# vlad17/runlmc

Hardware: AMD Instinct MI355X
Metric: kronecker_toeplitz_mvms_per_sec (higher is better)
Workload: dtype f64

## Files before the change

### runlmc_amd/csrc/rl_filter.h

```cpp
#pragma once
#include "rl_device.h"

#define RL_SF_G 512
#define RL_SF_NH (RL_SF_G / 256)
#define RL_SF_S 32
#define RL_SF_LPR (RL_SF_G / RL_SF_S)
#define RL_SF_PAD (RL_SF_G + RL_SF_LPR)
#define RL_SF_NSEG 32
#define RL_SF_MAXTOPS 16
#define RL_SF_TOL 2e-14

__device__ __forceinline__ int sf_pad(int i) { return i + (i >> 5); }

struct SfTop {
    double rho;
    double c[4];
    double rG;
    double rL;
};

struct SfParams {
    int NF, nfac;
    const SfTop* tops;
    const double* pw;
    const double* kappa;
    const double* facA;
    const double* facAW;
    const int* facJ;
    const double* pwp;
};

template <int NS>
__device__ __forceinline__ double sf_step(double (&F)[NS], double rho, double x) {
    const double tt = rho * F[0];
// ... 659 lines not shown
        const bool shifted = gi > m - 2;
#pragma unroll
        for (int k = 0; k < XR / 2; ++k)
            if (k < D) {
                const double p0 = shifted ? xr[2 * k + 1] : xr[2 * k];
                xs[(size_t)k * PAD + pi] = gi < m ? p0 : 0.0;
                xs[(size_t)k * PAD + pi + 1] = gi + 1 < m ? xr[2 * k + 1] : 0.0;
            }
    }
#pragma unroll
    for (int k = 0; k < 4; ++k)
        if (tid + 256 * k < ncin) cinl[tid + 256 * k] = cr[k];
    RL_SF_STAMP(101);
    if (nfac > 0) {
#pragma unroll
        for (int half = 0; half < NH; ++half) {
            const int pi = sf_pad(2 * tid) + half;
            double xb[D];
#pragma unroll
            for (int b = 0; b < D; ++b) xb[b] = xs[(size_t)b * PAD + pi];
            for (int f = 0; f < nfac; ++f) {
                const double* ar = facA + f * D;
                double u = 0.0;
#pragma unroll
                for (int b = 0; b < D; ++b) u = fma(ar[b], xb[b], u);
                us[(size_t)f * PAD + pi] = u;
            }
        }
    }
    sf_lds_barrier();
    RL_SF_STAMP(102);
}

template <int NS, int D>
static __global__ void __launch_bounds__(256) RL_SF_APPLY_ATTR
k_sf_apply(const double* __restrict__ X, double* __restrict__ Y, int nvec, int m, int NF,
           int nfac, const double* __restrict__ blob, const double* __restrict__ Cin,
           int* __restrict__ next_tile) {
    constexpr int G = RL_SF_G, PAD = RL_SF_PAD, NH = RL_SF_NH, XR = NH * D, S = RL_SF_S;
    constexpr int B2 = NS < 4 ? 2 : 1;
    RL_SMEM(smem);
    const int nchan = D * NF + nfac, nblob = sf_blob_doubles(NF, nfac, D);
    double* xs = reinterpret_cast<double*>(smem);
    double* us = xs + (size_t)D * PAD;
    double* tab = us + (size_t)nfac * PAD;
    const double* kap = tab;
    const double* facA = kap + NF * D;
    const double* facAW = facA + nfac * D;
    const double* facJ = facAW + nfac * D;
    const SfBlk* bl = reinterpret_cast<const SfBlk*>(facJ + nfac);
    double* cinl = tab + nblob;
    int* nxt = reinterpret_cast<int*>(cinl + (size_t)nchan * 2 * NS);
    double* scr = cinl + (size_t)nchan * 2 * NS + 1;
    const int tid = threadIdx.x, nthr = blockDim.x, lane = tid & 63, wave = tid >> 6;
    const int nwaves = nthr >> 6;
    RL_CENSUS_ENTER(120);
#if defined(RL_TIMING) && !defined(RL_EMU)
    const long long sf_t0 = wall_clock64();
#endif
    for (int e = tid; e < nblob; e += nthr) tab[e] = blob[e];
    sf_lds_barrier();
    const int nch = (m + G - 1) / G, ntiles = nch * nvec, ncin = nchan * 2 * NS;
    int tile = blockIdx.x, sf_iter = -1;
    if (tid == 0) nxt[0] = (int)gridDim.x + atomicAdd(next_tile, 1);
    if (tile < ntiles) {
        double xr[XR], cr[4];
        sf_request<XR>(xr, cr, X, Cin, tile, nch, nvec, D, m, ncin, tid);
        RL_SF_STAMP(100);
        sf_stage<D, XR>(xr, cr, xs, us, cinl, facA, nfac, ncin, (tile % nch) * G, m, tid, sf_iter);
    }
    int slot = 0;
    while (tile < ntiles) {
    const int chunk = tile % nch, v = tile / nch, g0 = chunk * G;
    ++sf_iter;
    RL_SF_STAMP(99);
    for (int t0 = 0; t0 < D * 16; t0 += nthr) {
#if !defined(RL_EMU)
        if (t0 + wave * 64 >= D * 16) break;
#endif
        const int t = t0 + tid, araw = t >> 4, s = t & 15;
#if defined(RL_EMU)
        const bool live = araw < D;
#else
        if (araw >= D) continue;
        constexpr bool live = true;
#endif
        const int a = live ? araw : D - 1;
        double* cell = xs + (size_t)a * PAD + s * (S + 1);
        double xv[S];
#pragma unroll
        for (int i = 0; i < S; ++i) xv[i] = cell[i];
        for (int j = 0; j < NF;) {
            const int b = (NS == 2 && NF - j >= 5) ? 5 : (NF - j >= B2 ? B2 : 1);
            const double* kw = kap + j * D + a;
            const double* cin0 = cinl + (size_t)(a * NF + j) * 2 * NS;
            if (j == 0) {
                if (NS == 2 && b == 5) sf_task<2, 5, true>(cell, xv, live, s, bl, j, kw, D, cin0, scr);
                else if (b == 2) sf_task<NS, B2, true>(cell, xv, live, s, bl, j, kw, D, cin0, scr);
                else sf_task<NS, 1, true>(cell, xv, live, s, bl, j, kw, D, cin0, scr);
            } else {
                if (NS == 2 && b == 5) sf_task<2, 5, false>(cell, xv, live, s, bl, j, kw, D, cin0, scr);
                else if (b == 2) sf_task<NS, B2, false>(cell, xv, live, s, bl, j, kw, D, cin0, scr);
                else sf_task<NS, 1, false>(cell, xv, live, s, bl, j, kw, D, cin0, scr);
            }
            j += b;
        }
    }
    RL_SF_STAMP(103);
    const int next = nxt[slot];
    double xr[XR], cr[4];
#if defined(RL_EMU)
    for (int k = 0; k < XR; ++k) xr[k] = 0.0;
    for (int k = 0; k < 4; ++k) cr[k] = 0.0;
#endif
    if (next < ntiles) sf_request<XR>(xr, cr, X, Cin, next, nch, nvec, D, m, ncin, tid);
    RL_SF_STAMP(104);
    const int xw = (D * 16 + 63) / 64, uw0 = xw < nwaves ? xw : 0, nuw = nwaves - uw0;
    for (int t0 = 0; t0 < nfac * 16; t0 += nuw * 64) {
        const int t = t0 + (wave - uw0) * 64 + lane, fraw = t >> 4, s = t & 15;
#if defined(RL_EMU)
        const bool live = wave >= uw0 && fraw < nfac;
#else
        if (wave < uw0 || fraw >= nfac) continue;
        constexpr bool live = true;
#endif
        const int f = live ? fraw : 0;
        double* cell = us + (size_t)f * PAD + s * (S + 1);
        double xv[S];
#pragma unroll
        for (int i = 0; i < S; ++i) xv[i] = cell[i];
        sf_task<NS, 1, true>(cell, xv, live, s, bl, (int)facJ[f], nullptr, 0,
                             cinl + (size_t)(D * NF + f) * 2 * NS, scr);
    }
    RL_SF_STAMP(110);
    sf_lds_barrier();
    RL_SF_STAMP(111);
    slot ^= 1;
    int drawn = 0;
    if (tid == 0 && next < ntiles) drawn = (int)gridDim.x + atomicAdd(next_tile, 1);
    {
        const double* gAW = facAW;
        const int i0 = 2 * tid, pi = sf_pad(i0);
        double* ybase = Y + (size_t)v * D * m + g0 + i0;
        double acc[NH][D];
#pragma unroll
        for (int half = 0; half < NH; ++half) {
#pragma unroll
            for (int a = 0; a < D; ++a) acc[half][a] = xs[(size_t)a * PAD + pi + half];
            for (int f = 0; f < nfac; ++f) {
                const double* ar = gAW + f * D;
                const double uw = us[(size_t)f * PAD + pi + half];
#pragma unroll
                for (int a = 0; a < D; ++a) acc[half][a] = fma(ar[a], uw, acc[half][a]);
            }
        }
        if (g0 + i0 + 1 < m) {
#pragma unroll
            for (int a = 0; a < D; ++a)
                *reinterpret_cast<SfPair*>(ybase + (size_t)a * m) = SfPair{acc[0][a], acc[1][a]};
        } else if (g0 + i0 < m) {
#pragma unroll
            for (int a = 0; a < D; ++a) ybase[(size_t)a * m] = acc[0][a];
        }
    }
    RL_SF_STAMP(112);
    if (tid == 0) nxt[slot] = drawn;
    tile = next;
    if (tile < ntiles) {
        RL_SF_STAMP(100);
        sf_stage<D, XR>(xr, cr, xs, us, cinl, facA, nfac, ncin, (tile % nch) * G, m, tid, sf_iter);
    }
    }
    RL_CENSUS_LEAVE(120);
#if defined(RL_TIMING) && !defined(RL_EMU)
    if (threadIdx.x == 0) {
        const unsigned long long d = (unsigned long long)(wall_clock64() - sf_t0);
        atomicMax((unsigned long long*)&rl_timing_buf[210], d);
        atomicAdd((unsigned long long*)&rl_timing_buf[211], d);
        atomicAdd((unsigned long long*)&rl_timing_buf[212], 1ull);
        atomicMax((unsigned long long*)&rl_timing_buf[213], (1ull << 40) - d);
    }
#endif
}
```

### runlmc_amd/csrc/rl_gridop.hip

```cpp
#include "rl_host.h"

static thread_local std::string g_err;

int fail(int code, const std::string& msg) {
    g_err = msg;
    return code;
}

extern "C" const char* rl_last_error(void) { return g_err.c_str(); }
extern "C" const char* rl_backend(void) { return RL_BACKEND_NAME; }
extern "C" int rl_abi_version(void) { return RL_ABI_VERSION; }
extern "C" int rl_device_count(int* count) {
    if (!count) return fail(RL_EINVAL, "count is NULL");
    RL_HIP(hipGetDeviceCount(count));
    return RL_OK;
}

void trace_once(const char* what) {
    static const bool on = getenv("RUNLMC_TRACE") != nullptr;
    if (!on) return;
    static std::vector<std::string> seen;
    for (const std::string& s : seen)
        if (s == what) return;
    seen.push_back(what);
// ... 29 lines not shown
        if (getenv(n) == nullptr) return false;
        if (!debug) ignored(n);
        return debug;
    };
    auto num = [&](const char* n, long long dflt) {
        const char* e = getenv(n);
        if (e == nullptr) return dflt;
        if (!debug) ignored(n);
        return debug ? atoll(e) : dflt;
    };
    k.pow2_only = user_flag("RUNLMC_POW2_ONLY");
    k.chunk_mb = (int)num("RUNLMC_CHUNK_MB", 0);
    k.two_streams = (int)num("RUNLMC_TWO_STREAMS", -1);
    k.affine = (int)num("RUNLMC_AFFINE", -1);
    k.affine_kb = (int)num("RUNLMC_AFFINE_KB", 0);
    k.affine_max_kb = (int)num("RUNLMC_AFFINE_MAX_KB", 2048);
    k.no_v1p = flag("RUNLMC_NO_V1P");
    k.v1p_min = (int)num("RUNLMC_V1P_MIN", 0);
    k.no_lowrank = flag("RUNLMC_NO_LOWRANK");
    k.no_filter = flag("RUNLMC_NO_FILTER");
    k.no_lr_bound = flag("RUNLMC_NO_LR_BOUND");
    k.sf_carries1 = flag("RUNLMC_SF_CARRIES1");
    k.sf_scan2 = flag("RUNLMC_SF_SCAN2");
    k.poly_round = flag("RUNLMC_POLY_ROUND");
    k.no_poly_round = flag("RUNLMC_NO_POLY_ROUND");
    k.lr_min = num("RUNLMC_LR_MIN", -1);
    k.staged_wt = flag("RUNLMC_STAGED_WT");
    k.no_staged_wt = flag("RUNLMC_NO_STAGED_WT");
    k.no_w_poly = flag("RUNLMC_NO_W_POLY");
    k.no_rp = flag("RUNLMC_NO_RP");
    k.rp_stagger = (int)num("RUNLMC_RP_STAGGER", 7);
    k.no_lr_small = flag("RUNLMC_NO_LR_SMALL");
    k.lr_expand_plain = (int)num("RUNLMC_LR_EXPAND_PLAIN", 0);
    k.no_precond_approx = flag("RUNLMC_NO_PRECOND_APPROX");
    k.no_precond_hi = flag("RUNLMC_NO_PRECOND_HI");
    k.precond_hi_passes = flag("RUNLMC_PRECOND_HI_PASSES");
    k.no_precond_hi_mixed = flag("RUNLMC_NO_PRECOND_HI_MIXED");
    k.precond_hi_min = num("RUNLMC_PRECOND_HI_MIN", 100000);
    k.precond_hi_rank = (int)num("RUNLMC_PRECOND_HI_RANK", 192);
    k.precond_hi_use = (int)num("RUNLMC_PRECOND_HI_USE", 0);
    k.rp_fly = (int)num("RUNLMC_RP_FLY", 1);
    k.no_rp_small = flag("RUNLMC_NO_RP_SMALL");
    k.no_rp_fuse = flag("RUNLMC_NO_RP_FUSE");
    k.rp_pfuse = !flag("RUNLMC_NO_RP_PFUSE");
    k.w_pfuse = !flag("RUNLMC_NO_W_PFUSE");
    k.rp_runlen = (int)num("RUNLMC_RP_RUNLEN", 0);
    k.w_poly_rmax = std::min(36, (int)num("RUNLMC_W_POLY_RMAX", 32));
    k.no_sort = flag("RUNLMC_NO_SORT");
    k.ws_cache_mb = user_num("RUNLMC_WS_CACHE_MB", -1);
    k.solver_maxblk = (int)num("RUNLMC_SOLVER_MAXBLK", 0);
    k.no_fuse_w = flag("RUNLMC_NO_FUSE_W");
    k.no_fuse_wt = flag("RUNLMC_NO_FUSE_WT");
    k.no_graph = flag("RUNLMC_NO_GRAPH");
#if defined(RL_EMU)
    k.minres_v1 = flag("RUNLMC_MINRES_V1");
#endif
    return k;
}

static int ilog2(int x) {
    int l = 0;
    while ((1 << l) < x) ++l;
    return l;
}

static FftPlan make_plan(int n) {
// ... 168 lines not shown
}

static void set_lds_attrs() {
#if !defined(RL_EMU)
    static unsigned long long seen = 0;
    if (!first_on_device(&seen)) return;
    (void)hipFuncSetAttribute((const void*)k_cols_fwd,
                              hipFuncAttributeMaxDynamicSharedMemorySize, 160 * 1024);
    (void)hipFuncSetAttribute((const void*)k_cols_inv,
                              hipFuncAttributeMaxDynamicSharedMemorySize, 160 * 1024);
    (void)hipFuncSetAttribute((const void*)k_rows_spec,
                              hipFuncAttributeMaxDynamicSharedMemorySize, 160 * 1024);
    set_lds_attr_cols2<8, 8>(); set_lds_attr_cols2<8, 16>(); set_lds_attr_cols2<16, 16>();
    set_lds_attr_cols2<3, 8>(); set_lds_attr_cols2<3, 16>();
    set_lds_attr_cols2<5, 8>(); set_lds_attr_cols2<5, 16>();
    set_lds_attr_rows<1>();  set_lds_attr_rows<2>();  set_lds_attr_rows<3>();
    set_lds_attr_rows<4>();  set_lds_attr_rows<5>();  set_lds_attr_rows<6>();
    set_lds_attr_rows<7>();  set_lds_attr_rows<8>();  set_lds_attr_rows<9>();
    set_lds_attr_rows<10>(); set_lds_attr_rows<11>(); set_lds_attr_rows<12>();
    set_lds_attr_rows<13>(); set_lds_attr_rows<14>(); set_lds_attr_rows<15>();
    set_lds_attr_rows<16>();
    set_lds_attr_rows3<1>();  set_lds_attr_rows3<2>();  set_lds_attr_rows3<3>();
    set_lds_attr_rows3<4>();  set_lds_attr_rows3<5>();  set_lds_attr_rows3<6>();
    set_lds_attr_rows3<7>();  set_lds_attr_rows3<8>();  set_lds_attr_rows3<9>();
    set_lds_attr_rows3<10>(); set_lds_attr_rows3<11>(); set_lds_attr_rows3<12>();
    set_lds_attr_rows3<13>(); set_lds_attr_rows3<14>(); set_lds_attr_rows3<15>();
    set_lds_attr_rows3<16>();
#define RL_SF_ATTR(D_)                                                                \
    (void)hipFuncSetAttribute((const void*)k_sf_apply<2, D_>,                         \
                              hipFuncAttributeMaxDynamicSharedMemorySize, 160 * 1024); \
    (void)hipFuncSetAttribute((const void*)k_sf_apply<3, D_>,                         \
                              hipFuncAttributeMaxDynamicSharedMemorySize, 160 * 1024); \
    (void)hipFuncSetAttribute((const void*)k_sf_apply<4, D_>,                         \
                              hipFuncAttributeMaxDynamicSharedMemorySize, 160 * 1024)
    RL_SF_ATTR(1); RL_SF_ATTR(2); RL_SF_ATTR(3); RL_SF_ATTR(4); RL_SF_ATTR(5); RL_SF_ATTR(6);
    RL_SF_ATTR(7); RL_SF_ATTR(8); RL_SF_ATTR(9); RL_SF_ATTR(10); RL_SF_ATTR(11); RL_SF_ATTR(12);
    RL_SF_ATTR(13); RL_SF_ATTR(14); RL_SF_ATTR(15); RL_SF_ATTR(16);
#undef RL_SF_ATTR
#define RL_LRS_ATTR(R_)                                                                      \
    (void)hipFuncSetAttribute((const void*)k_lr_small_project<R_>,                            \
                              hipFuncAttributeMaxDynamicSharedMemorySize, 160 * 1024);         \
    (void)hipFuncSetAttribute((const void*)k_lr_small_expand<R_>,                             \
                              hipFuncAttributeMaxDynamicSharedMemorySize, 160 * 1024)
    RL_LRS_ATTR(24); RL_LRS_ATTR(32); RL_LRS_ATTR(36); RL_LRS_ATTR(40); RL_LRS_ATTR(48);
#undef RL_LRS_ATTR
    (void)hipFuncSetAttribute((const void*)k_sf_carries<2>,
                              hipFuncAttributeMaxDynamicSharedMemorySize, 160 * 1024);
    (void)hipFuncSetAttribute((const void*)k_sf_carries<3>,
                              hipFuncAttributeMaxDynamicSharedMemorySize, 160 * 1024);
    (void)hipFuncSetAttribute((const void*)k_sf_carries<4>,
                              hipFuncAttributeMaxDynamicSharedMemorySize, 160 * 1024);
#endif
}


static unsigned div_magic(unsigned d);

template <int D>
static void launch1p_d(rl_gridop* g, unsigned pairs, hipStream_t st, const double* X, double* Y,
                       int nvec, int mode, const MixParams& mp, double* spec_out) {
#if !defined(RL_EMU)
    static unsigned long long seen = 0;
    if (first_on_device(&seen)) {
        (void)hipFuncSetAttribute((const void*)k1_product<D>,
                                  hipFuncAttributeMaxDynamicSharedMemorySize, 160 * 1024);
    }
// ... 900 lines not shown
        return;
    }
    lr_expand<R>(g, g->lr_zhat, nrows, Y, accumulate, st);
}

static int lr_apply(rl_gridop* g, const double* X, double* Y, int nvec, int q0, int Q,
                    const double* Bq, hipStream_t st) {
    const double* Cq = g->lr_C + (size_t)q0 * g->lr_r * g->lr_r;
    switch (g->lr_r) {
        case 24: lr_launch<24>(g, X, Y, nvec, Q, Cq, Bq, st); break;
        case 32: lr_launch<32>(g, X, Y, nvec, Q, Cq, Bq, st); break;
        case 36: lr_launch<36>(g, X, Y, nvec, Q, Cq, Bq, st); break;
        case 40: lr_launch<40>(g, X, Y, nvec, Q, Cq, Bq, st); break;
        case 48: lr_launch<48>(g, X, Y, nvec, Q, Cq, Bq, st); break;
        default: return fail(RL_EINVAL, "low-rank path: bad basis size");
    }
    RL_HIP(hipGetLastError());
    return RL_OK;
}

static int lr_apply_compact(rl_gridop* g, const double* X, double* Y, int nvec, hipStream_t st) {
    switch (g->lr_r) {
        case 24: lr_launch<24>(g, X, Y, nvec, g->lr_np, g->lr_Cc, g->lr_Bc, st, 1); break;
        case 32: lr_launch<32>(g, X, Y, nvec, g->lr_np, g->lr_Cc, g->lr_Bc, st, 1); break;
        case 36: lr_launch<36>(g, X, Y, nvec, g->lr_np, g->lr_Cc, g->lr_Bc, st, 1); break;
        case 40: lr_launch<40>(g, X, Y, nvec, g->lr_np, g->lr_Cc, g->lr_Bc, st, 1); break;
        case 48: lr_launch<48>(g, X, Y, nvec, g->lr_np, g->lr_Cc, g->lr_Bc, st, 1); break;
        default: return fail(RL_EINVAL, "low-rank path: bad basis size");
    }
    RL_HIP(hipGetLastError());
    return RL_OK;
}

static int mvm_with_mix(rl_gridop* g, const MixParams& mp, const double* X, double* Y, int nvec,
                        hipStream_t stream);

struct SfFit {
    int deg = 0;
    long double ah = 0.0L;
    long double c[4] = {0.0L, 0.0L, 0.0L, 0.0L};
};

static bool sf_check(const double* t, int m, const SfFit& f, long double tot) {
    const long double budget = (long double)RL_SF_TOL * tot, rho = expl(-f.ah);
    long double err = 0.0L, pw = 1.0L;
    for (int i = 0; i < m; ++i) {
        if ((i & 255) == 0) pw = expl(-f.ah * i);
        const long double model = (f.c[0] + (f.c[1] + (f.c[2] + f.c[3] * i) * i) * i) * pw;
        err += fabsl((long double)t[i] - model);
        if (!(err <= budget)) return false;
        pw *= rho;
    }
    return true;
}

static bool sf_detect(const double* t, int m, SfFit* fit) {
    if (m < 8) return false;
    long double tot = 0.0L;
    double amax = 0.0;
    int imax = 0;
    for (int i = 0; i < m; ++i) {
        if (!std::isfinite(t[i])) return false;
        const double a = std::fabs(t[i]);
        tot += a;
        if (a > amax) {
            amax = a;
// ... 102 lines not shown
           g->sf_Cin_cap >= sf_need_Cin(g, nvec, g->D * NF + nfac, NS);
}
static int sf_reserve(rl_gridop* g, int nvec, int NF, int nfac, int NS) {
    const size_t needE = sf_need_E(g, nvec, NF, NS), needC = sf_need_Cin(g, nvec, g->D * NF + nfac, NS);
    if (g->sf_E_cap < needE) {
        if (g->sf_E) RL_HIP(hipFree(g->sf_E));
        g->sf_E = nullptr;
        g->sf_E_cap = 0;
        RL_HIP(hipMalloc((void**)&g->sf_E, needE * sizeof(double)));
        g->sf_E_cap = needE;
    }
    if (g->sf_Cin_cap < needC) {
        if (g->sf_Cin) RL_HIP(hipFree(g->sf_Cin));
        g->sf_Cin = nullptr;
        g->sf_Cin_cap = 0;
        RL_HIP(hipMalloc((void**)&g->sf_Cin, needC * sizeof(double)));
        g->sf_Cin_cap = needC;
    }
    return RL_OK;
}
static size_t sf_apply_lds(int D, int nfac, int NF, int nthr, int NS) {
    size_t b = ((size_t)(D + nfac) * RL_SF_PAD + sf_blob_doubles(NF, nfac, D) +
                (size_t)(D * NF + nfac) * 2 * std::max(NS, 3) + 1) * sizeof(double);
#if defined(RL_EMU)
    b += (size_t)(nthr / 64) * 128 * sizeof(double);
#else
    (void)nthr;
#endif
    return b;
}

template <int NS>
static int sf_launch(rl_gridop* g, const SfParams& sp, const double* blob, const double* X,
                     double* Y, int nvec, hipStream_t st) {
    const int D = g->D, nrows = nvec * D, nch = sf_nchunks(g);
    if (D < 1 || D > 16) return fail(RL_ELIMIT, "filter form: D outside 1..16");
    const int rpw = nrows >= 16 * 64 ? 64 : 16;
    if (NS == 2 && !g->kn.sf_carries1)
        RL_LAUNCH(k_sf_carries2, dim3(nch, (nrows + rpw - 1) / rpw), dim3(256),
                  ((size_t)sp.NF * (RL_SF_G / 2) * 4 + 256) * sizeof(double), st, X, nrows, g->m,
                  sp.NF, sp.pwp, rpw, g->sf_E);
    else
        RL_LAUNCH((k_sf_carries<NS>), dim3(nch, (nrows + rpw - 1) / rpw), dim3(256),
                  ((size_t)sp.NF * (RL_SF_G + 1) + 256) * sizeof(double), st, X, nrows, g->m, sp.NF,
                  sp.pw, rpw, g->sf_E);
    const int ncd = 2 * (D * sp.NF + sp.nfac);
    if ((nch + RL_SF_NSEG - 1) / RL_SF_NSEG <= RL_SF_SEGMAX && !g->kn.sf_scan2)
        RL_LAUNCH((k_sf_scan1<NS>), dim3((ncd + 7) / 8, nvec), dim3(256), 256 * NS * sizeof(double),
                  st, (const double*)g->sf_E, nch, nvec, D, sp, g->sf_Cin, g->sf_next);
    else
        RL_LAUNCH((k_sf_scan<NS>), dim3((ncd + 7) / 8, nvec), dim3(256), 256 * NS * sizeof(double),
                  st, (const double*)g->sf_E, nch, nvec, D, sp, g->sf_Cin, g->sf_next);
    const int waves = 4;
#if defined(RL_EMU)
    const int ntiles = nch * nvec, resident = 7;
#else
    const size_t tile_lds = sf_apply_lds(D, sp.nfac, sp.NF, 256, NS);
    const int per_cu = (int)std::max<size_t>(1, std::min<size_t>(2, (160 * 1024) / tile_lds));
    const int ntiles = nch * nvec, resident = per_cu * RL_LR_CUS;
#endif
#define RL_SF_APPLY(D_)                                                                      \
    case D_:                                                                                    \
        RL_LAUNCH((k_sf_apply<NS, D_>), dim3(std::min(ntiles, resident)), dim3(64 * waves),     \
                  sf_apply_lds(D, sp.nfac, sp.NF, 64 * waves, NS), st, X, Y, nvec, g->m, sp.NF, \
                  sp.nfac, blob, (const double*)g->sf_Cin, g->sf_next);                         \
        break
    switch (D) {
        RL_SF_APPLY(1); RL_SF_APPLY(2); RL_SF_APPLY(3); RL_SF_APPLY(4);
        RL_SF_APPLY(5); RL_SF_APPLY(6); RL_SF_APPLY(7); RL_SF_APPLY(8);
        RL_SF_APPLY(9); RL_SF_APPLY(10); RL_SF_APPLY(11); RL_SF_APPLY(12);
        RL_SF_APPLY(13); RL_SF_APPLY(14); RL_SF_APPLY(15); RL_SF_APPLY(16);
        default: return fail(RL_ELIMIT, "filter form: no k_sf_apply for this D");
    }
#undef RL_SF_APPLY
    RL_HIP(hipGetLastError());
    return RL_OK;
}

static int sf_apply_all(rl_gridop* g, const double* X, double* Y, int nvec, hipStream_t st) {
    SfParams sp{g->sf_n, g->sf_nfac, g->sf_tops, g->sf_pw, g->sf_kappa, g->sf_facA, g->sf_facAW,
                g->sf_facJ, g->sf_pwp};
    switch (g->sf_ns) {
        case 4: return sf_launch<4>(g, sp, g->sf_blob, X, Y, nvec, st);
        case 3: return sf_launch<3>(g, sp, g->sf_blob, X, Y, nvec, st);
        default: return sf_launch<2>(g, sp, g->sf_blob, X, Y, nvec, st);
    }
}
static int sf_apply_top(rl_gridop* g, int q, const double* X, double* Y, int nvec, hipStream_t st) {
    const int j = g->sf_slot[q];
    SfParams sp{1, 0, g->sf_tops + j, g->sf_pw + (size_t)j * (RL_SF_G + 1), g->ones, nullptr,
                nullptr, nullptr, g->sf_pwp + (size_t)j * 2 * RL_SF_G};
    const double* blob = g->sf_blob_top + (size_t)j * sf_blob_doubles(1, 0, g->D);
    switch (g->sf_top_ns[q]) {
        case 4: return sf_launch<4>(g, sp, blob, X, Y, nvec, st);
        case 3: return sf_launch<3>(g, sp, blob, X, Y, nvec, st);
        default: return sf_launch<2>(g, sp, blob, X, Y, nvec, st);
    }
}

__global__ void __launch_bounds__(256)
k_lr_finish_C(const double* __restrict__ part, int nparts, int nrows, int r,
              const double* __restrict__ nu, double* __restrict__ C) {
    RL_SMEM(smem);
    double* red = reinterpret_cast<double*>(smem);
    const int i = blockIdx.x, j = threadIdx.x & 63, cls = threadIdx.x >> 6;
    double a = 0.0, b = 0.0;
    if (j < r)
        for (int c = cls; c < nparts; c += 4) {
            a += part[((size_t)c * nrows + j) * r + i];
            b += part[((size_t)c * nrows + i) * r + j];
        }
    red[cls * 64 + j] = a;
    red[256 + cls * 64 + j] = b;
    __syncthreads();
    if (cls == 0 && j < r) {
        a = (red[j] + red[64 + j]) + (red[128 + j] + red[192 + j]);
        b = (red[256 + j] + red[320 + j]) + (red[384 + j] + red[448 + j]);
        C[i * r + j] = 0.5 * (nu[i] * a + nu[j] * b);
    }
// ... 643 lines not shown
        g->defer_expand = false;
        const int rc = lr_ensure(g);
        g->defer_expand = defer;
        if (rc != RL_OK) return rc;
    }
    if (big && !g->lr_dirty) {
        const bool single = mp.nfac == 0 && mp.Q == 1 && mp.kappa == g->ones;
        const int q1 = single ? (int)((mp.spec - g->spec) / g->L) : -1;
        const int form = single ? g->top_form[q1] : (g->lr_ok ? 1 : (g->st_ok ? 3 : 0));
        const bool poly_part = form == 1 || (form == 3 && g->lr_np > 0);
        bool ready = true;
        if (poly_part)
            ready = g->lr_part_cap >= lr_part_need(g, nvec) &&
                    g->lr_zhat_cap >= (size_t)nvec * g->D * RL_LR_RMAX;
        const int sNF = single ? 1 : g->sf_n, sfac = single ? 0 : g->sf_nfac;
        const int sNS = single ? (form == 2 ? g->sf_top_ns[q1] : 2) : g->sf_ns;
        if (form >= 2) ready = ready && sf_ready(g, nvec, sNF, sfac, sNS);
        if (form != 0 && !ready && !capturing) {
            if (poly_part) RL_TRY(lr_reserve(g, nvec));
            if (form >= 2) RL_TRY(sf_reserve(g, nvec, sNF, sfac, sNS));
            ready = true;
        }
        if (form != 0 && ready) {
            if (form == 1) {
                trace_once("grid product: polynomial-subspace form (k_lr_project / mix / expand)");
                if (single) return lr_apply(g, X, Y, nvec, q1, 1, g->lr_eye, stream);
                return lr_apply(g, X, Y, nvec, 0, g->Q, g->lr_B, stream);
            }
            if (form == 2) {
                trace_once("grid product: recursive-filter form (k_sf_carries / scan / apply)");
                return sf_apply_top(g, q1, X, Y, nvec, stream);
            }
            trace_once("grid product: recursive-filter part + polynomial part");
            RL_TRY(sf_apply_all(g, X, Y, nvec, stream));
            if (g->lr_np > 0) RL_TRY(lr_apply_compact(g, X, Y, nvec, stream));
            return RL_OK;
        }
    }
    const bool small_try = !big && g->lr_try && !g->lr_bypass && !g->kn.no_lr_small &&
                           (size_t)g->D * g->m <= RL_LR_SMALL_MAX && g->lr_min == lr_min_elements(g) &&
                           !(mp.nfac == 0 && mp.Q == 1 && mp.kappa == g->ones);
    if (small_try && g->lr_dirty && !stream_capturing(stream)) RL_TRY(lr_ensure(g));
    if (small_try && !g->lr_dirty && g->lr_ok && g->lr_Mf_ok && nvec <= 65535) {
        const int nseg = lr_small_nseg(g->m);
        const size_t need = (size_t)nvec * g->D * nseg * RL_LR_RMAX;
        if (g->lr_spart_cap < need && !stream_capturing(stream)) {
            if (g->lr_spart) RL_HIP(hipFree(g->lr_spart));
            g->lr_spart = nullptr;
            g->lr_spart_cap = 0;
            RL_HIP(hipMalloc((void**)&g->lr_spart, need * sizeof(double)));
            g->lr_spart_cap = need;
        }
        if (g->lr_spart_cap >= need) {
            trace_once("grid product: polynomial-subspace form, small batch (k_lr_small_project / k_lr_small_expand)");
            const dim3 grid(g->D * nseg, nvec), blk(RL_LR_SMALL_WG);
#define RL_LR_SMALL(R_)                                                                           \
            RL_LAUNCH(k_lr_small_project<R_>, grid, blk, lr_small_project_lds(R_), stream, X, g->D, g->m, nseg, \
                      (const double*)g->lr_beta, g->lr_spart);                                     \
            RL_LAUNCH(k_lr_small_expand<R_>, grid, blk, lr_small_expand_lds(g->D, R_), stream,     \
                      (const double*)g->lr_spart, g->D, g->m, nseg, (const double*)g->lr_beta,     \
                      (const double*)g->lr_Mf, Y)
            switch (g->lr_r) {
                case 24: RL_LR_SMALL(24); break;
                case 32: RL_LR_SMALL(32); break;
                case 36: RL_LR_SMALL(36); break;
                case 40: RL_LR_SMALL(40); break;
// ... 179 lines not shown
```

### runlmc_amd/csrc/rl_host.h

```cpp
#pragma once
#include "../../include/runlmc_hip.h"

#include <algorithm>
#include <cmath>
#include <cstdio>
#include <cstdlib>
#include <cstring>
#include <functional>
#include <string>
#include <thread>
#include <vector>

#include "rl_kernels.h"
#include "rl_kernels2.h"
#include "rl_kernels3.h"
#include "rl_lowrank.h"
#include "rl_rowpoly.h"
#include "rl_filter.h"

#define RL_MAX_D 16

int fail(int code, const std::string& msg);
#define RL_HIP(expr)                                                                   \
    do {                                                                               \
// ... 11 lines not shown

void trace_once(const char* what);
bool first_on_device(unsigned long long* seen);

struct RlKnobs {
    bool pow2_only = false;
    int chunk_mb = 0;
    int two_streams = -1;
    int affine = -1;
    int affine_kb = 0;
    int affine_max_kb = 2048;
    bool no_v1p = false;
    int v1p_min = 0;
    bool no_lowrank = false;
    bool no_filter = false;
    bool sf_scan2 = false;
    bool sf_carries1 = false;
    bool no_lr_bound = false;
    bool poly_round = false;
    bool no_poly_round = false;
    long long lr_min = -1;
    bool staged_wt = false;
    bool no_staged_wt = false;
    bool no_w_poly = false;
    bool no_rp = false;
    int rp_stagger = 7;
    int rp_runlen = 0;
    bool no_rp_small = false;
    bool rp_pfuse = true;
    bool w_pfuse = true;
    bool no_rp_fuse = false;
    bool no_lr_small = false;
    int lr_expand_plain = 0;
    bool no_precond_approx = false;
    long long precond_hi_min = 100000;
    int precond_hi_use = 0;
    int precond_hi_rank = 192;
    bool no_precond_hi_mixed = false;
    bool precond_hi_passes = false;
    bool no_precond_hi = false;
    int rp_fly = 1;
    int w_poly_rmax = 32;
    bool no_sort = false;
    long long ws_cache_mb = -1;
    int solver_maxblk = 0;
    bool no_fuse_w = false;
    bool no_fuse_wt = false;
    bool no_graph = false;
    bool minres_v1 = false;
};
RlKnobs read_knobs();

template <class T>
static int upload(T** dev, const std::vector<T>& host) {
    RL_HIP(hipMalloc((void**)dev, std::max<size_t>(host.size(), 1) * sizeof(T)));
    if (!host.empty())
        RL_HIP(hipMemcpy(*dev, host.data(), host.size() * sizeof(T), hipMemcpyHostToDevice));
    return RL_OK;
}

static const size_t kLdsSoft = 76 * 1024;
static const size_t kLdsHard = 156 * 1024;

struct rl_gridop {
    RlKnobs kn;
    int device = 0;
// ... 295 lines not shown
```

### runlmc_amd/csrc/rl_lowrank.h

```cpp
#pragma once
#include "rl_device.h"

#define RL_LR_RMAX 48
#define RL_LR_T 32
#define RL_LR_WAVES 4
#define RL_LR_CUS 256
#define RL_LR_RB(R) ((R) <= 24 ? 4 : 2)
#define RL_LR_G(R) ((R) <= 24 ? 2 : 4)
#define RL_LR_ROWS(R) (RL_LR_RB(R) * RL_LR_WAVES)
#if defined(RL_EMU)
#define RL_LR_PROJECT_ATTR
#define RL_LR_UNIFORM(x) (x)
#else
#define RL_LR_PROJECT_ATTR __attribute__((amdgpu_waves_per_eu(2)))
#define RL_LR_UNIFORM(x) __builtin_amdgcn_readfirstlane(x)
#endif
#define RL_LR_TOL 2e-13

__device__ __forceinline__ int lr_slots(int m) { return (m + 1) / 2; }
__device__ __forceinline__ double lr_point(int n, int m) {
    return m > 1 ? fma(2.0 / (double)(m - 1), (double)n, -1.0) : 0.0;
}

template <int R>
// ... 286 lines not shown
        if (live) *y0 = (ev + od) + o0;
        if (pair) *y1 = (ev - od) + o1;
    }
}

struct LrLinesGrid {
    int nbx, nby, rpb, period;
};
static inline int lr_expand_rpb(int nbx, int nr, int ncls, int rpb_max, int round_wgs) {
    if (rpb_max > 0 &&
        (size_t)nbx * ncls * ((nr + rpb_max - 1) / rpb_max) >= (size_t)2 * round_wgs)
        return rpb_max;
    int nby = round_wgs / (nbx * ncls);
    nby = nby < nr ? nby : nr;
    nby = nby > 1 ? nby : 1;
    return (nr + nby - 1) / nby;
}
static inline LrLinesGrid lr_expand_lines_grid(int nrows, int m, int rpb_max, int round_wgs) {
    LrLinesGrid g;
    int gcd = 16;
    while ((m & 15) % gcd != 0) gcd >>= 1;
    g.period = 16 / gcd;
    g.nbx = ((m + 1) / 2 + 15 + 255) / 256;
    const int ncr = (nrows + g.period - 1) / g.period;
    g.rpb = lr_expand_rpb(g.nbx, ncr, g.period, rpb_max, round_wgs);
    g.nby = g.period * ((ncr + g.rpb - 1) / g.rpb);
    return g;
}
template <int R>
static void lr_expand_launch(const double* zhat, int nrows, int m, const double* beta, double* Y,
                             bool accumulate, int rpb_max, int round_wgs, int plain,
                             hipStream_t st, bool pad8 = true) {
    const int p0 = (int)((reinterpret_cast<unsigned long long>(Y) >> 3) & 15ull);
    const bool measured = R < 36 && !accumulate;
    if ((plain != 0 && plain != 3) || (plain == 0 && !measured) || ((m & 15) == 0 && p0 == 0)) {
        const int nbx = ((m + 1) / 2 + 255) / 256;
        const int rpb = lr_expand_rpb(nbx, nrows, 1, rpb_max, round_wgs);
        const int nby = (nrows + rpb - 1) / rpb;
        const dim3 grid(nbx, plain == 2 ? (nby + 7) / 8 * 8 : nby);
        if (accumulate)
            RL_LAUNCH((k_lr_expand<R, true>), grid, dim3(256), 0, st, zhat, nrows, m, beta, rpb, Y);
        else
            RL_LAUNCH((k_lr_expand<R, false>), grid, dim3(256), 0, st, zhat, nrows, m, beta, rpb, Y);
        return;
    }
    const LrLinesGrid g = lr_expand_lines_grid(nrows, m, rpb_max, round_wgs);
    const dim3 grid(g.nbx, pad8 ? (g.nby + 7) / 8 * 8 : g.nby);
    if (accumulate)
        RL_LAUNCH((k_lr_expand_lines<R, true>), grid, dim3(256), 0, st, zhat, nrows, m, beta, g.rpb,
                  g.period, g.nby, Y);
    else
        RL_LAUNCH((k_lr_expand_lines<R, false>), grid, dim3(256), 0, st, zhat, nrows, m, beta, g.rpb,
                  g.period, g.nby, Y);
}

#define RL_LR_SMALL_MAX 32768
#define RL_LR_SMALL_WG 256
#define RL_LR_SU 4
#define RL_LR_SMP 32
static inline int lr_small_nseg(int m) {
    const int slots = (m + 1) / 2;
    int nseg = (slots + RL_LR_SMALL_WG * RL_LR_SU - 1) / (RL_LR_SMALL_WG * RL_LR_SU);
    return nseg < 1 ? 1 : (nseg > 16 ? 16 : nseg);
}
template <int R>
__global__ void __launch_bounds__(RL_LR_SMALL_WG)
k_lr_small_project(const double* __restrict__ X, int D, int m, int nseg, const double* __restrict__ beta,
// ... 328 lines not shown
```

Baseline: 308,800.

## Fuse polynomial low-rank expansion into recursive-filter apply kernel

Computes low-rank coefficients (project+mix) first, then has the filter apply kernel evaluate the three-term polynomial recurrence per point and add the low-rank contribution into its accumulators before writing Y. This removes the separate low-rank expand pass and its read-modify-write of Y. Coefficients are double-buffered in LDS and prefetched per tile; fusion is only enabled when the extra LDS does not reduce per-CU residency. Also lets the lines-style expand path be used for larger ranks when not accumulating.

```diff
diff --git a/runlmc_amd/csrc/rl_filter.h b/runlmc_amd/csrc/rl_filter.h
--- a/runlmc_amd/csrc/rl_filter.h
+++ b/runlmc_amd/csrc/rl_filter.h
@@ -1,5 +1,6 @@
 #pragma once
 #include "rl_device.h"
+#include "rl_lowrank.h"
 
 #define RL_SF_G 512
 #define RL_SF_NH (RL_SF_G / 256)
@@ -725,13 +726,41 @@
     RL_SF_STAMP(102);
 }
 
-template <int NS, int D>
+__host__ __device__ inline int sf_zrow(int D) { return (D + 1) & ~1; }
+__host__ __device__ inline int sf_poly_doubles(int D, int pr) {
+    return pr > 0 ? 2 * pr * sf_zrow(D) + pr + 1 : 0;
+}
+struct __attribute__((aligned(16))) SfPair16 {
+    double a, b;
+};
+template <int ZK>
+__device__ __forceinline__ void sf_request_z(double (&zr)[ZK], const double* __restrict__ Zhat,
+                                             int v, int dr, int tid) {
+    const double* src = Zhat + (size_t)v * dr;
+#pragma unroll
+    for (int k = 0; k < ZK; ++k) zr[k] = src[tid + 256 * k < dr ? tid + 256 * k : dr - 1];
+}
+template <int D, int ZK>
+__device__ __forceinline__ void sf_stage_z(const double (&zr)[ZK], double* zb, int pr, int tid) {
+#pragma unroll
+    for (int k = 0; k < ZK; ++k) {
+        const int e = tid + 256 * k;
+        if (e < D * pr) {
+            const int a = e / pr, j = e - a * pr;
+            zb[j * sf_zrow(D) + a] = zr[k];
+        }
+    }
+}
+
+template <int NS, int D, bool POLY = false>
 static __global__ void __launch_bounds__(256) RL_SF_APPLY_ATTR
 k_sf_apply(const double* __restrict__ X, double* __restrict__ Y, int nvec, int m, int NF,
            int nfac, const double* __restrict__ blob, const double* __restrict__ Cin,
-           int* __restrict__ next_tile) {
+           int* __restrict__ next_tile, int pr, const double* __restrict__ Zhat,
+           const double* __restrict__ beta) {
     constexpr int G = RL_SF_G, PAD = RL_SF_PAD, NH = RL_SF_NH, XR = NH * D, S = RL_SF_S;
     constexpr int B2 = NS < 4 ? 2 : 1;
+    constexpr int ZD = (D + 1) & ~1, ZK = POLY ? (D * RL_LR_RMAX + 255) / 256 : 1;
     RL_SMEM(smem);
     const int nchan = D * NF + nfac, nblob = sf_blob_doubles(NF, nfac, D);
     double* xs = reinterpret_cast<double*>(smem);
@@ -747,6 +776,18 @@
     double* scr = cinl + (size_t)nchan * 2 * NS + 1;
     const int tid = threadIdx.x, nthr = blockDim.x, lane = tid & 63, wave = tid >> 6;
     const int nwaves = nthr >> 6;
+    double* zl = nullptr;
+    const double* betal = nullptr;
+    if constexpr (POLY) {
+        size_t zoff = (size_t)(cinl - xs) + (size_t)nchan * 2 * (NS > 3 ? NS : 3) + 1;
+#if defined(RL_EMU)
+        zoff += (size_t)nwaves * 128;
+#endif
+        zl = xs + ((zoff + 1) & ~(size_t)1);
+        double* bw = zl + (size_t)2 * pr * ZD;
+        for (int e = tid; e < pr; e += nthr) bw[e] = beta[e];
+        betal = bw;
+    }
     RL_CENSUS_ENTER(120);
 #if defined(RL_TIMING) && !defined(RL_EMU)
     const long long sf_t0 = wall_clock64();
@@ -759,10 +800,15 @@
     if (tile < ntiles) {
         double xr[XR], cr[4];
         sf_request<XR>(xr, cr, X, Cin, tile, nch, nvec, D, m, ncin, tid);
+        if constexpr (POLY) {
+            double zr[ZK];
+            sf_request_z<ZK>(zr, Zhat, tile / nch, D * pr, tid);
+            sf_stage_z<D, ZK>(zr, zl, pr, tid);
+        }
         RL_SF_STAMP(100);
         sf_stage<D, XR>(xr, cr, xs, us, cinl, facA, nfac, ncin, (tile % nch) * G, m, tid, sf_iter);
     }
-    int slot = 0;
+    int slot = 0, zcur = 0;
     while (tile < ntiles) {
     const int chunk = tile % nch, v = tile / nch, g0 = chunk * G;
     ++sf_iter;
@@ -807,6 +853,13 @@
     for (int k = 0; k < 4; ++k) cr[k] = 0.0;
 #endif
     if (next < ntiles) sf_request<XR>(xr, cr, X, Cin, next, nch, nvec, D, m, ncin, tid);
+    double zr[ZK];
+    if constexpr (POLY) {
+#if defined(RL_EMU)
+        for (int k = 0; k < ZK; ++k) zr[k] = 0.0;
+#endif
+        if (next < ntiles) sf_request_z<ZK>(zr, Zhat, next / nch, D * pr, tid);
+    }
     RL_SF_STAMP(104);
     const int xw = (D * 16 + 63) / 64, uw0 = xw < nwaves ? xw : 0, nuw = nwaves - uw0;
     for (int t0 = 0; t0 < nfac * 16; t0 += nuw * 64) {
@@ -847,6 +900,45 @@
                 for (int a = 0; a < D; ++a) acc[half][a] = fma(ar[a], uw, acc[half][a]);
             }
         }
+        if constexpr (POLY) {
+            const double* zc = zl + (size_t)zcur * pr * ZD;
+            const int n0 = g0 + i0;
+            const double s0 = lr_point(n0 < m ? n0 : m - 1, m);
+            const double s1 = lr_point(n0 + 1 < m ? n0 + 1 : m - 1, m);
+            double q0 = 1.0, q1 = 1.0, qm0 = 0.0, qm1 = 0.0;
+            constexpr int ZU = D <= 10 ? 4 : 2;
+            for (int j4 = 0; j4 < pr; j4 += ZU) {
+                SfPair16 z[ZU][ZD / 2];
+                double b[ZU];
+#pragma unroll
+                for (int u = 0; u < ZU; ++u) {
+#pragma unroll
+                    for (int a = 0; a < ZD / 2; ++a)
+                        z[u][a] = *reinterpret_cast<const SfPair16*>(zc + (j4 + u) * ZD + 2 * a);
+                    b[u] = betal[j4 + u];
+                }
+#if !defined(RL_EMU)
+                __builtin_amdgcn_sched_barrier(0);
+#endif
+#pragma unroll
+                for (int u = 0; u < ZU; ++u) {
+#pragma unroll
+                    for (int a = 0; a < D; a += 2) {
+                        acc[0][a] = fma(z[u][a / 2].a, q0, acc[0][a]);
+                        acc[1][a] = fma(z[u][a / 2].a, q1, acc[1][a]);
+                        if (a + 1 < D) {
+                            acc[0][a + 1] = fma(z[u][a / 2].b, q0, acc[0][a + 1]);
+                            acc[1][a + 1] = fma(z[u][a / 2].b, q1, acc[1][a + 1]);
+                        }
+                    }
+                    const double qn0 = fma(s0, q0, -b[u] * qm0), qn1 = fma(s1, q1, -b[u] * qm1);
+                    qm0 = q0;
+                    qm1 = q1;
+                    q0 = qn0;
+                    q1 = qn1;
+                }
+            }
+        }
         if (g0 + i0 + 1 < m) {
 #pragma unroll
             for (int a = 0; a < D; ++a)
@@ -859,6 +951,13 @@
     RL_SF_STAMP(112);
     if (tid == 0) nxt[slot] = drawn;
     tile = next;
+    if constexpr (POLY) {
+        zcur ^= 1;
+        if (tile < ntiles) sf_stage_z<D, ZK>(zr, zl + (size_t)zcur * pr * ZD, pr, tid);
+    } else {
+        (void)zr;
+        (void)zcur;
+    }
     if (tile < ntiles) {
         RL_SF_STAMP(100);
         sf_stage<D, XR>(xr, cr, xs, us, cinl, facA, nfac, ncin, (tile % nch) * G, m, tid, sf_iter);
diff --git a/runlmc_amd/csrc/rl_gridop.hip b/runlmc_amd/csrc/rl_gridop.hip
--- a/runlmc_amd/csrc/rl_gridop.hip
+++ b/runlmc_amd/csrc/rl_gridop.hip
@@ -85,6 +85,7 @@
     k.rp_stagger = (int)num("RUNLMC_RP_STAGGER", 7);
     k.no_lr_small = flag("RUNLMC_NO_LR_SMALL");
     k.lr_expand_plain = (int)num("RUNLMC_LR_EXPAND_PLAIN", 0);
+    k.sf_poly_fuse = (int)num("RUNLMC_SF_POLY_FUSE", 1);
     k.no_precond_approx = flag("RUNLMC_NO_PRECOND_APPROX");
     k.no_precond_hi = flag("RUNLMC_NO_PRECOND_HI");
     k.precond_hi_passes = flag("RUNLMC_PRECOND_HI_PASSES");
@@ -319,6 +320,10 @@
     (void)hipFuncSetAttribute((const void*)k_sf_apply<3, D_>,                         \
                               hipFuncAttributeMaxDynamicSharedMemorySize, 160 * 1024); \
     (void)hipFuncSetAttribute((const void*)k_sf_apply<4, D_>,                         \
+                              hipFuncAttributeMaxDynamicSharedMemorySize, 160 * 1024); \
+    (void)hipFuncSetAttribute((const void*)k_sf_apply<2, D_, true>,                   \
+                              hipFuncAttributeMaxDynamicSharedMemorySize, 160 * 1024); \
+    (void)hipFuncSetAttribute((const void*)k_sf_apply<3, D_, true>,                   \
                               hipFuncAttributeMaxDynamicSharedMemorySize, 160 * 1024)
     RL_SF_ATTR(1); RL_SF_ATTR(2); RL_SF_ATTR(3); RL_SF_ATTR(4); RL_SF_ATTR(5); RL_SF_ATTR(6);
     RL_SF_ATTR(7); RL_SF_ATTR(8); RL_SF_ATTR(9); RL_SF_ATTR(10); RL_SF_ATTR(11); RL_SF_ATTR(12);
@@ -1285,6 +1290,24 @@
     return RL_OK;
 }
 
+template <int R>
+static void lr_coeffs(rl_gridop* g, const double* X, int nvec, hipStream_t st) {
+    const int chunks = lr_project<R>(g, X, nvec * g->D, st);
+    lr_mix<R>(g, g->lr_part, chunks, nvec, g->lr_np, g->lr_Cc, g->lr_Bc, g->lr_zhat, st);
+}
+static int lr_coeffs_compact(rl_gridop* g, const double* X, int nvec, hipStream_t st) {
+    switch (g->lr_r) {
+        case 24: lr_coeffs<24>(g, X, nvec, st); break;
+        case 32: lr_coeffs<32>(g, X, nvec, st); break;
+        case 36: lr_coeffs<36>(g, X, nvec, st); break;
+        case 40: lr_coeffs<40>(g, X, nvec, st); break;
+        case 48: lr_coeffs<48>(g, X, nvec, st); break;
+        default: return fail(RL_EINVAL, "low-rank path: bad basis size");
+    }
+    RL_HIP(hipGetLastError());
+    return RL_OK;
+}
+
 static int mvm_with_mix(rl_gridop* g, const MixParams& mp, const double* X, double* Y, int nvec,
                         hipStream_t stream);
 
@@ -1453,9 +1476,11 @@
 
 template <int NS>
 static int sf_launch(rl_gridop* g, const SfParams& sp, const double* blob, const double* X,
-                     double* Y, int nvec, hipStream_t st) {
+                     double* Y, int nvec, hipStream_t st, int pr = 0, const double* zhat = nullptr,
+                     const double* beta = nullptr) {
     const int D = g->D, nrows = nvec * D, nch = sf_nchunks(g);
     if (D < 1 || D > 16) return fail(RL_ELIMIT, "filter form: D outside 1..16");
+    if (pr > 0 && NS > 3) return fail(RL_EINVAL, "filter form: no polynomial part with four states");
     const int rpw = nrows >= 16 * 64 ? 64 : 16;
     if (NS == 2 && !g->kn.sf_carries1)
         RL_LAUNCH(k_sf_carries2, dim3(nch, (nrows + rpw - 1) / rpw), dim3(256),
@@ -1476,15 +1501,23 @@
 #if defined(RL_EMU)
     const int ntiles = nch * nvec, resident = 7;
 #else
-    const size_t tile_lds = sf_apply_lds(D, sp.nfac, sp.NF, 256, NS);
+    const size_t tile_lds = sf_apply_lds(D, sp.nfac, sp.NF, 256, NS) + sf_poly_doubles(D, pr) * sizeof(double);
     const int per_cu = (int)std::max<size_t>(1, std::min<size_t>(2, (160 * 1024) / tile_lds));
     const int ntiles = nch * nvec, resident = per_cu * RL_LR_CUS;
 #endif
+    const size_t lds = sf_apply_lds(D, sp.nfac, sp.NF, 64 * waves, NS) + sf_poly_doubles(D, pr) * sizeof(double);
+#define RL_SF_APPLY_K(K_)                                                                      \
+    RL_LAUNCH((K_), dim3(std::min(ntiles, resident)), dim3(64 * waves), lds, st, X, Y, nvec,    \
+              g->m, sp.NF, sp.nfac, blob, (const double*)g->sf_Cin, g->sf_next, pr, zhat, beta)
 #define RL_SF_APPLY(D_)                                                                      \
     case D_:                                                                                    \
-        RL_LAUNCH((k_sf_apply<NS, D_>), dim3(std::min(ntiles, resident)), dim3(64 * waves),     \
-                  sf_apply_lds(D, sp.nfac, sp.NF, 64 * waves, NS), st, X, Y, nvec, g->m, sp.NF, \
-                  sp.nfac, blob, (const double*)g->sf_Cin, g->sf_next);                         \
+        if constexpr (NS <= 3) {                                                                \
+            if (pr > 0) {                                                                       \
+                RL_SF_APPLY_K((k_sf_apply<NS, D_, true>));                                      \
+                break;                                                                          \
+            }                                                                                   \
+        }                                                                                       \
+        RL_SF_APPLY_K((k_sf_apply<NS, D_, false>));                                             \
         break
     switch (D) {
         RL_SF_APPLY(1); RL_SF_APPLY(2); RL_SF_APPLY(3); RL_SF_APPLY(4);
@@ -1494,18 +1527,29 @@
         default: return fail(RL_ELIMIT, "filter form: no k_sf_apply for this D");
     }
 #undef RL_SF_APPLY
+#undef RL_SF_APPLY_K
     RL_HIP(hipGetLastError());
     return RL_OK;
 }
 
-static int sf_apply_all(rl_gridop* g, const double* X, double* Y, int nvec, hipStream_t st) {
+static int sf_apply_all(rl_gridop* g, const double* X, double* Y, int nvec, hipStream_t st,
+                        int pr = 0) {
     SfParams sp{g->sf_n, g->sf_nfac, g->sf_tops, g->sf_pw, g->sf_kappa, g->sf_facA, g->sf_facAW,
                 g->sf_facJ, g->sf_pwp};
+    const double* zhat = pr > 0 ? g->lr_zhat : nullptr;
+    const double* beta = pr > 0 ? g->lr_beta : nullptr;
     switch (g->sf_ns) {
         case 4: return sf_launch<4>(g, sp, g->sf_blob, X, Y, nvec, st);
-        case 3: return sf_launch<3>(g, sp, g->sf_blob, X, Y, nvec, st);
-        default: return sf_launch<2>(g, sp, g->sf_blob, X, Y, nvec, st);
-    }
+        case 3: return sf_launch<3>(g, sp, g->sf_blob, X, Y, nvec, st, pr, zhat, beta);
+        default: return sf_launch<2>(g, sp, g->sf_blob, X, Y, nvec, st, pr, zhat, beta);
+    }
+}
+static bool sf_poly_fused(const rl_gridop* g) {
+    if (!g->kn.sf_poly_fuse || g->lr_np <= 0 || g->sf_ns > 3) return false;
+    const size_t base = sf_apply_lds(g->D, g->sf_nfac, g->sf_n, 256, g->sf_ns);
+    const size_t fused = base + sf_poly_doubles(g->D, g->lr_r) * sizeof(double);
+    const size_t lds = 160 * 1024;
+    return fused <= kLdsHard && std::min<size_t>(2, lds / fused) == std::min<size_t>(2, lds / base);
 }
 static int sf_apply_top(rl_gridop* g, int q, const double* X, double* Y, int nvec, hipStream_t st) {
     const int j = g->sf_slot[q];
@@ -2215,6 +2259,10 @@
                 return sf_apply_top(g, q1, X, Y, nvec, stream);
             }
             trace_once("grid product: recursive-filter part + polynomial part");
+            if (sf_poly_fused(g)) {
+                RL_TRY(lr_coeffs_compact(g, X, nvec, stream));
+                return sf_apply_all(g, X, Y, nvec, stream, g->lr_r);
+            }
             RL_TRY(sf_apply_all(g, X, Y, nvec, stream));
             if (g->lr_np > 0) RL_TRY(lr_apply_compact(g, X, Y, nvec, stream));
             return RL_OK;
diff --git a/runlmc_amd/csrc/rl_host.h b/runlmc_amd/csrc/rl_host.h
--- a/runlmc_amd/csrc/rl_host.h
+++ b/runlmc_amd/csrc/rl_host.h
@@ -67,6 +67,7 @@
     bool no_rp_fuse = false;
     bool no_lr_small = false;
     int lr_expand_plain = 0;
+    int sf_poly_fuse = 1;
     bool no_precond_approx = false;
     long long precond_hi_min = 100000;
     int precond_hi_use = 0;
diff --git a/runlmc_amd/csrc/rl_lowrank.h b/runlmc_amd/csrc/rl_lowrank.h
--- a/runlmc_amd/csrc/rl_lowrank.h
+++ b/runlmc_amd/csrc/rl_lowrank.h
@@ -342,7 +342,7 @@
                              bool accumulate, int rpb_max, int round_wgs, int plain,
                              hipStream_t st, bool pad8 = true) {
     const int p0 = (int)((reinterpret_cast<unsigned long long>(Y) >> 3) & 15ull);
-    const bool measured = R < 36 && !accumulate;
+    const bool measured = !accumulate;
     if ((plain != 0 && plain != 3) || (plain == 0 && !measured) || ((m & 15) == 0 && p0 == 0)) {
         const int nbx = ((m + 1) / 2 + 255) / 256;
         const int rpb = lr_expand_rpb(nbx, nrows, 1, rpb_max, round_wgs);
```

After: 286,000. 0.926x the previous value.
